# cure-lab/MagicDrive

Hardware: NVIDIA H100
Metric: 6-view 224x400 denoising-steps/sec (higher is better)
Workload: dtype bf16

## Files before the change

### magicdrive_b200/csrc/attention_wgmma.cuh

```cuda
#pragma once
#include "ptx.cuh"
#include "wgmma.cuh"

namespace mdb {

constexpr int ATT_BM = 128;

constexpr int ATT_MAX_SRC = 3;
struct AttnKvMaps {
  CUtensorMap k[ATT_MAX_SRC], v[ATT_MAX_SRC];
};

struct AttnParams {
  void* out;
  int ldo;
  int lq, lk;
  const int* kv_index;
  int n_sets;
  const int* kv_len;
  int n_src;
  float scale_log2;
  int q_step;
};

template <int D, int BN_ = 0>
struct AttnCfg {
  static constexpr int KD = (D + 63) / 64;
  static constexpr int D16 = (D + 15) / 16 * 16;
  static constexpr int BN = BN_ ? BN_ : ((D16 <= 64) ? 128 : 64);
  static constexpr int TILE_Q = ATT_BM * 128;
  static constexpr int TILE_KV = BN * 128;
  static constexpr int SMEM_Q = KD * TILE_Q;
  static constexpr int STAGES_FIT = (232448 - 1024 - 256 - SMEM_Q) / (2 * KD * TILE_KV);
  static constexpr int STAGES = STAGES_FIT > 4 ? 4 : STAGES_FIT;
  static constexpr int SMEM_KV = STAGES * 2 * KD * TILE_KV;
  static constexpr int kSmemBytes = SMEM_Q + SMEM_KV + 1024 + 256;
  static constexpr int kConsumerWarps = 8;
  static constexpr int kThreads = 32 * kConsumerWarps + 32;
  static constexpr int SACC = BN / 2;
  static constexpr int OACC = D16 / 2;
  static_assert(STAGES >= 1 && kSmemBytes <= 232448, "shared memory");
};

template <int D, int BN_, bool CAUSAL = false, bool KVRES = false, bool F16 = false>
__global__ void __launch_bounds__(AttnCfg<D, BN_>::kThreads, 1)
attention_wgmma_kernel(const __grid_constant__ CUtensorMap tmQ, const __grid_constant__ AttnKvMaps kvm, const AttnParams p) {
  using Cfg = AttnCfg<D, BN_>;
  using A = Act<F16>;
  using Elt = typename A::T;
  constexpr int KD = Cfg::KD, D16 = Cfg::D16, BN = Cfg::BN, STAGES = Cfg::STAGES;
  constexpr int TILE_Q = Cfg::TILE_Q, TILE_KV = Cfg::TILE_KV;
  extern __shared__ uint8_t smem_raw[];
  uint8_t* smem = reinterpret_cast<uint8_t*>((reinterpret_cast<uintptr_t>(smem_raw) + 1023) & ~uintptr_t(1023));
  uint8_t* smQ = smem;
  uint8_t* smK = smQ + Cfg::SMEM_Q;
  uint8_t* smV = smK + STAGES * KD * TILE_KV;
  uint64_t* bars = reinterpret_cast<uint64_t*>(smV + STAGES * KD * TILE_KV);
  uint64_t* q_full = bars;
  uint64_t* q_empty = bars + 1;
  uint64_t* kv_full = bars + 2;
  uint64_t* kv_empty = bars + 2 + STAGES;

  const int warp = threadIdx.x >> 5, lane = threadIdx.x & 31;
  const int b = blockIdx.z, head = blockIdx.y;
  const int nq = (p.lq + ATT_BM - 1) / ATT_BM;
  const int q_step = p.q_step > 0 ? p.q_step : nq;
  const int n_own = (nq - static_cast<int>(blockIdx.x) + q_step - 1) / q_step;
  auto q0_of = [&](int o) { return (static_cast<int>(blockIdx.x) + o * q_step) * ATT_BM; };

  if (warp == Cfg::kConsumerWarps && lane == 0) {
    prefetch_tmap(&tmQ);
    for (int i = 0; i < p.n_src; ++i) {
      prefetch_tmap(&kvm.k[i]);
      prefetch_tmap(&kvm.v[i]);
    }
    mbar_init(q_full, 1);
    mbar_init(q_empty, Cfg::kConsumerWarps);
    for (int i = 0; i < STAGES; ++i) {
      mbar_init(&kv_full[i], 1);
      mbar_init(&kv_empty[i], Cfg::kConsumerWarps);
    }
    fence_barrier_init();
  }
  __syncthreads();
  asm volatile("griddepcontrol.wait;" ::: "memory");
  asm volatile("griddepcontrol.launch_dependents;" ::: "memory");
  const int lkb = p.kv_len ? min(max(p.kv_len[b], 0), p.lk) : p.lk;
  const int ntiles = (lkb + BN - 1) / BN;
  static_assert(!(CAUSAL && KVRES), "resident key tiles: every query tile walks all of them");
  const bool kv_resident = (KVRES ? ntiles <= STAGES : ntiles == 1) && p.n_sets == 1 && n_own > 1;
  auto kv_entry = [&](int set) { return p.kv_index ? p.kv_index[b * p.n_sets + set] : b; };
  auto tiles_of = [&](int kve, int q0) {
    return kve < 0 ? 0 : CAUSAL ? min(ntiles, (min(q0 + ATT_BM, p.lq) - 1) / BN + 1) : ntiles;
  };

  if (warp == Cfg::kConsumerWarps) {
    if (lane == 0) {
      int stage = 0;
      uint32_t phase = 0;
      for (int o = 0; o < n_own; ++o) {
        if (o > 0) mbar_wait(q_empty, static_cast<uint32_t>(o - 1) & 1u);
        mbar_arrive_expect_tx(q_full, KD * TILE_Q);
#pragma unroll
        for (int c = 0; c < KD; ++c) tma_load_4d(&tmQ, q_full, smQ + c * TILE_Q, c * 64, head, q0_of(o), b);
        if (kv_resident && o > 0) continue;
        for (int set = 0; set < p.n_sets; ++set) {
          const int kve = kv_entry(set);
          const int nt = tiles_of(kve, q0_of(o));
          if (nt == 0) continue;
          const int kvb = kve & 0xffffff;
          const CUtensorMap* km = &kvm.k[kve >> 24];
          const CUtensorMap* vm = &kvm.v[kve >> 24];
          for (int j = 0; j < nt; ++j) {
            mbar_wait(&kv_empty[stage], phase ^ 1);
            mbar_arrive_expect_tx(&kv_full[stage], 2 * KD * TILE_KV);
#pragma unroll
            for (int c = 0; c < KD; ++c) {
              tma_load_4d(km, &kv_full[stage], smK + (stage * KD + c) * TILE_KV, c * 64, head, j * BN, kvb);
              tma_load_4d(vm, &kv_full[stage], smV + (stage * KD + c) * TILE_KV, c * 64, head, j * BN, kvb);
            }
            if (++stage == STAGES) {
              stage = 0;
              phase ^= 1;
            }
          }
        }
      }
    }
    return;
  }

  const int wg = warp >> 2;
  const int q = lane & 3;
  const int rloc = 64 * wg + 16 * (warp & 3) + (lane >> 2);
  const float sc = p.scale_log2;
  int stage = 0;
  uint32_t phase = 0;
  for (int o = 0; o < n_own; ++o) {
    const int q0 = q0_of(o);
    mbar_wait(q_full, static_cast<uint32_t>(o) & 1u);
    bool wrote = false;
    for (int set = 0; set < p.n_sets; ++set) {
      const int nt = tiles_of(kv_entry(set), q0);
      if (nt == 0) continue;
      float oacc[Cfg::OACC];
#pragma unroll
      for (int i = 0; i < Cfg::OACC; ++i) oacc[i] = 0.f;
      float m[2] = {-INFINITY, -INFINITY}, l[2] = {0.f, 0.f};
      for (int j = 0; j < nt; ++j) {
        const int st = kv_resident ? (KVRES ? j : 0) : stage;
        mbar_wait(&kv_full[st], kv_resident ? 0u : phase);
        float s[Cfg::SACC];
        wgmma_fence();
#pragma unroll
        for (int k = 0; k < D16 / 16; ++k) {
          const int c = k / 4, kk = k % 4;
          const uint64_t adesc = make_sw128_kmajor_desc(smem_u32(smQ + c * TILE_Q + wg * (64 * 128))) + 2 * kk;
          const uint64_t bdesc = make_sw128_kmajor_desc(smem_u32(smK + (st * KD + c) * TILE_KV)) + 2 * kk;
          WgmmaSS<BN, F16>::run(s, adesc, bdesc, k > 0 ? 1u : 0u);
        }
        wgmma_commit();
        wgmma_wait<0>();
        const int kbase = j * BN;
        if (kbase + BN > lkb) {
#pragma unroll
          for (int g = 0; g < BN / 8; ++g)
#pragma unroll
            for (int e = 0; e < 2; ++e)
              if (kbase + 8 * g + 2 * q + e >= lkb) s[4 * g + e] = s[4 * g + 2 + e] = -INFINITY;
        }
        if constexpr (CAUSAL) {
          if (kbase + BN - 1 > q0 + rloc) {
#pragma unroll
            for (int g = 0; g < BN / 8; ++g)
#pragma unroll
              for (int h = 0; h < 2; ++h)
#pragma unroll
                for (int e = 0; e < 2; ++e)
                  if (kbase + 8 * g + 2 * q + e > q0 + rloc + 8 * h) s[4 * g + 2 * h + e] = -INFINITY;
          }
        }
        float corr[2];
#pragma unroll
        for (int h = 0; h < 2; ++h) {
          float mx = -INFINITY;
#pragma unroll
          for (int g = 0; g < BN / 8; ++g) mx = fmaxf(mx, fmaxf(s[4 * g + 2 * h], s[4 * g + 2 * h + 1]));
          mx = fmaxf(mx, __shfl_xor_sync(0xffffffffu, mx, 1));
          mx = fmaxf(mx, __shfl_xor_sync(0xffffffffu, mx, 2));
          const float m_new = fmaxf(m[h], mx * sc);
          corr[h] = exp2f(m[h] - m_new);
          m[h] = m_new;
        }
        uint32_t pa[BN / 16][4];
        float rs[2] = {0.f, 0.f};
#pragma unroll
        for (int kk = 0; kk < BN / 16; ++kk) {
#pragma unroll
          for (int r = 0; r < 4; ++r) {
            const int h = r & 1;
            const int i0 = 8 * kk + 4 * (r >> 1) + 2 * h;
            const float p0 = exp2f(fmaf(s[i0], sc, -m[h]));
            const float p1 = exp2f(fmaf(s[i0 + 1], sc, -m[h]));
            rs[h] += p0 + p1;
            pa[kk][r] = A::pack(p0, p1);
          }
        }
#pragma unroll
        for (int h = 0; h < 2; ++h) l[h] = l[h] * corr[h] + rs[h];
#pragma unroll
        for (int g = 0; g < D16 / 8; ++g) {
          oacc[4 * g] *= corr[0], oacc[4 * g + 1] *= corr[0];
          oacc[4 * g + 2] *= corr[1], oacc[4 * g + 3] *= corr[1];
        }
        wgmma_fence();
#pragma unroll
        for (int kk = 0; kk < BN / 16; ++kk) {
          const uint64_t bdesc = make_sw128_mnmajor_desc(smem_u32(smV + st * KD * TILE_KV), TILE_KV) + (2048u >> 4) * kk;
          WgmmaRSBmn<D16, F16>::run(oacc, pa[kk], bdesc, 1u);
        }
        wgmma_commit();
        wgmma_wait<0>();
        if (!kv_resident) {
          if (lane == 0) mbar_arrive(&kv_empty[stage]);
          if (++stage == STAGES) {
            stage = 0;
            phase ^= 1;
          }
        }
      }
#pragma unroll
      for (int h = 0; h < 2; ++h) {
        l[h] += __shfl_xor_sync(0xffffffffu, l[h], 1);
        l[h] += __shfl_xor_sync(0xffffffffu, l[h], 2);
      }
      const float inv[2] = {1.0f / l[0], 1.0f / l[1]};
#pragma unroll
      for (int h = 0; h < 2; ++h) {
        const int qrow = q0 + rloc + 8 * h;
        if (qrow >= p.lq) continue;
        Elt* orow = static_cast<Elt*>(p.out) + (static_cast<long long>(b) * p.lq + qrow) * p.ldo + head * D;
#pragma unroll
        for (int g = 0; g < D16 / 8; ++g) {
          const int col = 8 * g + 2 * q;
          if (col >= D) continue;
          float f0 = oacc[4 * g + 2 * h] * inv[h], f1 = oacc[4 * g + 2 * h + 1] * inv[h];
          if (wrote) {
            const float2 pf = A::to_float2(*reinterpret_cast<const typename A::T2*>(orow + col));
            f0 = A::to_float(A::from_float(f0)) + pf.x;
            f1 = A::to_float(A::from_float(f1)) + pf.y;
          }
          *reinterpret_cast<uint32_t*>(orow + col) = A::pack(f0, f1);
        }
      }
      wrote = true;
    }
    if (!wrote) {
#pragma unroll
      for (int h = 0; h < 2; ++h) {
        const int qrow = q0 + rloc + 8 * h;
        if (qrow >= p.lq) continue;
        Elt* orow = static_cast<Elt*>(p.out) + (static_cast<long long>(b) * p.lq + qrow) * p.ldo + head * D;
#pragma unroll
        for (int g = 0; g < D16 / 8; ++g)
          if (8 * g + 2 * q < D) *reinterpret_cast<uint32_t*>(orow + 8 * g + 2 * q) = 0u;
      }
    }
    __syncwarp();
    if (lane == 0) mbar_arrive(q_empty);
  }
}

}
```

### magicdrive_b200/csrc/capi_attention.cu

```cuda
#include <cuda_bf16.h>
#include <cuda_runtime.h>

#include <stdlib.h>
#include <string.h>

#include "../../include/magicdrive_b200.h"
#define MDB_NEED_TENSORMAP
#include "common_host.h"
#include "attention_wgmma.cuh"

namespace {

bool make_qkv_map(CUtensorMap* m, const void* ptr, int d, int heads, int l, int b, int ld, int rows, bool f16) {
  mdb::EncodeTiledFn enc = mdb::get_encode();
  if (!enc) return false;
  cuuint64_t dims[4] = {(cuuint64_t)d, (cuuint64_t)heads, (cuuint64_t)l, (cuuint64_t)b};
  cuuint64_t strides[3] = {(cuuint64_t)d * 2, (cuuint64_t)ld * 2, (cuuint64_t)l * ld * 2};
  cuuint32_t box[4] = {64u, 1u, (cuuint32_t)rows, 1u};
  cuuint32_t estr[4] = {1u, 1u, 1u, 1u};
  return enc(m, f16 ? CU_TENSOR_MAP_DATA_TYPE_FLOAT16 : CU_TENSOR_MAP_DATA_TYPE_BFLOAT16, 4, const_cast<void*>(ptr), dims, strides, box, estr,
             CU_TENSOR_MAP_INTERLEAVE_NONE, CU_TENSOR_MAP_SWIZZLE_128B, CU_TENSOR_MAP_L2_PROMOTION_L2_256B,
             CU_TENSOR_MAP_FLOAT_OOB_FILL_NONE) == CUDA_SUCCESS;
}

struct KvSources {
  const void* k[mdb::ATT_MAX_SRC];
  const void* v[mdb::ATT_MAX_SRC];
  int ldk[mdb::ATT_MAX_SRC], ldv[mdb::ATT_MAX_SRC], b_kv[mdb::ATT_MAX_SRC];
  int n;
};

bool make_kv_maps(mdb::AttnKvMaps* m, const KvSources& s, int d, int heads, int lk, int rows, bool f16) {
  for (int i = 0; i < mdb::ATT_MAX_SRC; ++i) {
    const int j = i < s.n ? i : 0;
    if (!make_qkv_map(&m->k[i], s.k[j], d, heads, lk, s.b_kv[j], s.ldk[j], rows, f16) ||
        !make_qkv_map(&m->v[i], s.v[j], d, heads, lk, s.b_kv[j], s.ldv[j], rows, f16))
      return false;
  }
  return true;
}

int attn_num_sms() {
  static int sms = 0;
  if (!sms) {
    int dev = 0;
    cudaGetDevice(&dev);
    if (cudaDeviceGetAttribute(&sms, cudaDevAttrMultiProcessorCount, dev) != cudaSuccess || sms <= 0) sms = 132;
  }
  return sms;
}

int multi_q_step(int b, int heads, int lq, int lk, int n_sets, int bn, bool resident) {
  if ((lk > bn && !resident) || n_sets != 1) return 0;
  const char* e = getenv("MDB_ATTN_MULTIQ");
  if (e && e[0] == '0') return 0;
  const int nq = (lq + mdb::ATT_BM - 1) / mdb::ATT_BM;
  const long long per_tile_ctas = static_cast<long long>(b) * heads;
  const long long slots = attn_num_sms();
  if (per_tile_ctas * nq <= slots) return 0;
  long long gx = slots / per_tile_ctas;
  if (gx < 1) gx = 1;
  if (gx >= nq) return 0;
  return static_cast<int>(gx);
}

constexpr int ATT_RESIDENT_MAX_LK = 256;

template <int D, int BN_, bool CAUSAL, bool KVRES = false, bool F16 = false>
int launch_attention(const void* q, int ldq, const KvSources& src, void* out, int ldo, int b, int heads, int lq, int lk,
                     const int* kv_index, int n_sets, const int* kv_len, float scale, cudaStream_t st) {
  using Cfg = mdb::AttnCfg<D, BN_>;
  if constexpr (!CAUSAL && !KVRES) {
    if (kv_len && n_sets == 1 && lk <= ATT_RESIDENT_MAX_LK)
      return launch_attention<D, BN_, false, true, F16>(q, ldq, src, out, ldo, b, heads, lq, lk, kv_index, n_sets, kv_len, scale, st);
  }
  static bool attr = false;
  if (!attr) {
    cudaError_t e = cudaFuncSetAttribute(mdb::attention_wgmma_kernel<D, BN_, CAUSAL, KVRES, F16>, cudaFuncAttributeMaxDynamicSharedMemorySize, Cfg::kSmemBytes);
    if (e != cudaSuccess) return mdb::set_error(MDB_ERR_CUDA, "attention_wgmma_kernel smem attr: %s", cudaGetErrorString(e));
    attr = true;
  }
  CUtensorMap tq;
  mdb::AttnKvMaps kvm;
  if (!make_qkv_map(&tq, q, D, heads, lq, b, ldq, mdb::ATT_BM, F16) || !make_kv_maps(&kvm, src, D, heads, lk, Cfg::BN, F16))
    return mdb::set_error(MDB_ERR_CUDA, "mdb_attention: cuTensorMapEncodeTiled failed (d=%d heads=%d lq=%d lk=%d)", D, heads, lq, lk);
  mdb::AttnParams p;
  p.out = out;
  p.ldo = ldo, p.lq = lq, p.lk = lk, p.kv_index = kv_index, p.n_sets = n_sets, p.kv_len = kv_len, p.n_src = src.n;
  p.scale_log2 = scale * 1.4426950408889634f;
  p.q_step = multi_q_step(b, heads, lq, lk, n_sets, Cfg::BN, KVRES);
  dim3 grid(p.q_step > 0 ? p.q_step : (lq + mdb::ATT_BM - 1) / mdb::ATT_BM, heads, b);
  cudaError_t le = mdb::launch_pdl(mdb::attention_wgmma_kernel<D, BN_, CAUSAL, KVRES, F16>, grid, dim3(Cfg::kThreads), Cfg::kSmemBytes, st, tq, kvm, p);
  if (le != cudaSuccess) return mdb::set_error(MDB_ERR_CUDA, "attention_wgmma_kernel launch: %s", cudaGetErrorString(le));
  cudaError_t e2 = cudaGetLastError();
  if (e2 != cudaSuccess) return mdb::set_error(MDB_ERR_CUDA, "attention_wgmma_kernel: %s", cudaGetErrorString(e2));
  return MDB_OK;
}

template <int BN_, bool CAUSAL, bool F16 = false>
int attention_dispatch_bn(const void* q, int ldq, const KvSources& src, void* out, int ldo, int b, int heads, int lq, int lk, int d,
                          const int* kv_index, int n_sets, const int* kv_len, float scale, cudaStream_t st) {
  switch (d) {
    case 32: return launch_attention<32, BN_, CAUSAL, false, F16>(q, ldq, src, out, ldo, b, heads, lq, lk, kv_index, n_sets, kv_len, scale, st);
    case 40: return launch_attention<40, BN_, CAUSAL, false, F16>(q, ldq, src, out, ldo, b, heads, lq, lk, kv_index, n_sets, kv_len, scale, st);
    case 64: return launch_attention<64, BN_, CAUSAL, false, F16>(q, ldq, src, out, ldo, b, heads, lq, lk, kv_index, n_sets, kv_len, scale, st);
    case 80: return launch_attention<80, BN_, CAUSAL, false, F16>(q, ldq, src, out, ldo, b, heads, lq, lk, kv_index, n_sets, kv_len, scale, st);
    case 160: return launch_attention<160, BN_, CAUSAL, false, F16>(q, ldq, src, out, ldo, b, heads, lq, lk, kv_index, n_sets, kv_len, scale, st);
    default: return mdb::set_error(MDB_ERR_UNSUPPORTED, "mdb_attention: head dim %d not instantiated (32, 40, 64, 80, 160)", d);
  }
}

template <bool CAUSAL = false>
int attention_dispatch(const void* q, int ldq, const KvSources& src, void* out, int ldo, int b, int heads, int lq, int lk, int d,
                       const int* kv_index, int n_sets, const int* kv_len, float scale, cudaStream_t st) {
  const char* e = getenv("MDB_ATTN_KERNEL");
  if (e && !strcmp(e, "tc2d")) return attention_dispatch_bn<64, CAUSAL>(q, ldq, src, out, ldo, b, heads, lq, lk, d, kv_index, n_sets, kv_len, scale, st);
  if (e && !strcmp(e, "tc")) return attention_dispatch_bn<128, CAUSAL>(q, ldq, src, out, ldo, b, heads, lq, lk, d, kv_index, n_sets, kv_len, scale, st);
  if (e && *e && strcmp(e, "tc2"))
    return mdb::set_error(MDB_ERR_INVALID, "mdb_attention: MDB_ATTN_KERNEL must be tc2, tc2d or tc (got %s)", e);
  return attention_dispatch_bn<0, CAUSAL>(q, ldq, src, out, ldo, b, heads, lq, lk, d, kv_index, n_sets, kv_len, scale, st);
}

template <bool F16>
int attention_varlen(const void* q, int ldq, int n_src, const void* const* k, const int* ldk, const void* const* v,
                     const int* ldv, const int* b_kv, void* out, int ldo, int b, int heads, int lq, int lk, int d,
                     const int* kv_index, int n_sets, const int* kv_len, float scale, void* stream) {
  using namespace mdb;
  if (!q || !k || !v || !ldk || !ldv || !b_kv || !out) return set_error(MDB_ERR_INVALID, "mdb_attention: null pointer");
  if (n_src < 1 || n_src > ATT_MAX_SRC) return set_error(MDB_ERR_INVALID, "mdb_attention: 1..%d K/V sources", ATT_MAX_SRC);
  if (n_sets < 1 || n_sets > MDB_ATT_MAX_SETS || (n_sets > 1 && !kv_index))
    return set_error(MDB_ERR_INVALID, "mdb_attention: n_sets must be 1..%d (more than 1 needs kv_index)", MDB_ATT_MAX_SETS);
  if (scale <= 0.f) return set_error(MDB_ERR_INVALID, "mdb_attention: scale must be positive");
  if (lq <= 0 || lk <= 0 || b <= 0 || heads <= 0) return set_error(MDB_ERR_INVALID, "mdb_attention: bad shape");
  if (ldq % 8 || ldo % 8) return set_error(MDB_ERR_UNSUPPORTED, "mdb_attention: strides must be multiples of 8");
  KvSources src;
  src.n = n_src;
  for (int i = 0; i < n_src; ++i) {
    if (!k[i] || !v[i] || b_kv[i] <= 0) return set_error(MDB_ERR_INVALID, "mdb_attention: bad K/V source %d", i);
    if (ldk[i] % 8 || ldv[i] % 8) return set_error(MDB_ERR_UNSUPPORTED, "mdb_attention: strides must be multiples of 8");
    src.k[i] = k[i], src.v[i] = v[i], src.ldk[i] = ldk[i], src.ldv[i] = ldv[i], src.b_kv[i] = b_kv[i];
  }
  if (!kv_index && (n_src != 1 || b_kv[0] != b)) return set_error(MDB_ERR_INVALID, "mdb_attention: b_kv != b or several sources need kv_index");
  if constexpr (F16) {
    return attention_dispatch_bn<0, false, true>(q, ldq, src, out, ldo, b, heads, lq, lk, d, kv_index, n_sets, kv_len, scale,
                                                 static_cast<cudaStream_t>(stream));
  } else {
    return attention_dispatch(q, ldq, src, out, ldo, b, heads, lq, lk, d, kv_index, n_sets, kv_len, scale,
                              static_cast<cudaStream_t>(stream));
  }
}

}

extern "C" int mdb_attention_varlen(const void* q, int ldq, int n_src, const void* const* k, const int* ldk, const void* const* v,
                                    const int* ldv, const int* b_kv, void* out, int ldo, int b, int heads, int lq, int lk, int d,
                                    const int* kv_index, int n_sets, const int* kv_len, float scale, void* stream) {
  return attention_varlen<false>(q, ldq, n_src, k, ldk, v, ldv, b_kv, out, ldo, b, heads, lq, lk, d, kv_index, n_sets, kv_len,
                                 scale, stream);
}

extern "C" int mdb_attention_varlen_f16(const void* q, int ldq, int n_src, const void* const* k, const int* ldk,
                                        const void* const* v, const int* ldv, const int* b_kv, void* out, int ldo, int b, int heads,
                                        int lq, int lk, int d, const int* kv_index, int n_sets, const int* kv_len, float scale,
                                        void* stream) {
  return attention_varlen<true>(q, ldq, n_src, k, ldk, v, ldv, b_kv, out, ldo, b, heads, lq, lk, d, kv_index, n_sets, kv_len,
                                scale, stream);
}

extern "C" int mdb_attention_multi(const void* q, int ldq, int n_src, const void* const* k, const int* ldk, const void* const* v,
                                   const int* ldv, const int* b_kv, void* out, int ldo, int b, int heads, int lq, int lk, int d,
                                   const int* kv_index, int n_sets, float scale, void* stream) {
  return mdb_attention_varlen(q, ldq, n_src, k, ldk, v, ldv, b_kv, out, ldo, b, heads, lq, lk, d, kv_index, n_sets, nullptr, scale,
                              stream);
}

extern "C" int mdb_attention(const void* q, int ldq, const void* k, int ldk, const void* v, int ldv, void* out, int ldo, int b,
                             int b_kv, int heads, int lq, int lk, int d, const int* kv_index, int n_sets, float scale,
                             void* stream) {
  return mdb_attention_multi(q, ldq, 1, &k, &ldk, &v, &ldv, &b_kv, out, ldo, b, heads, lq, lk, d, kv_index, n_sets, scale, stream);
}

extern "C" int mdb_attention_causal(const void* q, int ldq, const void* k, int ldk, const void* v, int ldv, void* out, int ldo,
                                    int b, int heads, int lq, int lk, int d, float scale, void* stream) {
  using namespace mdb;
  if (!q || !k || !v || !out) return set_error(MDB_ERR_INVALID, "mdb_attention_causal: null pointer");
  if (lq != lk) return set_error(MDB_ERR_INVALID, "mdb_attention_causal: lq (%d) must equal lk (%d)", lq, lk);
  if (scale <= 0.f) return set_error(MDB_ERR_INVALID, "mdb_attention_causal: scale must be positive");
  if (lq <= 0 || b <= 0 || heads <= 0) return set_error(MDB_ERR_INVALID, "mdb_attention_causal: bad shape");
  if (ldq % 8 || ldk % 8 || ldv % 8 || ldo % 8) return set_error(MDB_ERR_UNSUPPORTED, "mdb_attention_causal: strides must be multiples of 8");
  KvSources src;
  src.n = 1;
  src.k[0] = k, src.v[0] = v, src.ldk[0] = ldk, src.ldv[0] = ldv, src.b_kv[0] = b;
  return attention_dispatch<true>(q, ldq, src, out, ldo, b, heads, lq, lk, d, nullptr, 1, nullptr, scale,
                                  static_cast<cudaStream_t>(stream));
}
```

Measured before the change: 59.06.

## Add persistent attention kernel with double-buffered Q tiles

Adds a persistent variant of the WGMMA attention kernel that launches at most one CTA per SM and walks a flattened list of (batch, head, query-tile) work items in strides. Q is double-buffered in shared memory so the producer warp can load the next tile's Q and K/V while consumers finish the current one. The goal is to cut per-CTA launch and prologue cost and hide tile-boundary latency. In exchange it drops the resident-KV reuse path for these launches, needs extra shared memory, and may balance load worse when item counts do not divide evenly across SMs.

```diff
diff --git a/magicdrive_b200/csrc/attention_wgmma.cuh b/magicdrive_b200/csrc/attention_wgmma.cuh
--- a/magicdrive_b200/csrc/attention_wgmma.cuh
+++ b/magicdrive_b200/csrc/attention_wgmma.cuh
@@ -1,6 +1,8 @@
 #pragma once
 #include "ptx.cuh"
 #include "wgmma.cuh"
+
+#include <type_traits>
 
 namespace mdb {
 
@@ -21,6 +23,9 @@
   int n_src;
   float scale_log2;
   int q_step;
+};
+struct AttnParamsPersist : AttnParams {
+  int heads, b;
 };
 
 template <int D, int BN_ = 0>
@@ -35,6 +40,7 @@
   static constexpr int STAGES = STAGES_FIT > 4 ? 4 : STAGES_FIT;
   static constexpr int SMEM_KV = STAGES * 2 * KD * TILE_KV;
   static constexpr int kSmemBytes = SMEM_Q + SMEM_KV + 1024 + 256;
+  static constexpr int kSmemBytesPersist = kSmemBytes + SMEM_Q;
   static constexpr int kConsumerWarps = 8;
   static constexpr int kThreads = 32 * kConsumerWarps + 32;
   static constexpr int SACC = BN / 2;
@@ -42,30 +48,38 @@
   static_assert(STAGES >= 1 && kSmemBytes <= 232448, "shared memory");
 };
 
-template <int D, int BN_, bool CAUSAL = false, bool KVRES = false, bool F16 = false>
+template <int D, int BN_, bool CAUSAL = false, bool KVRES = false, bool F16 = false, bool PERSIST = false>
 __global__ void __launch_bounds__(AttnCfg<D, BN_>::kThreads, 1)
-attention_wgmma_kernel(const __grid_constant__ CUtensorMap tmQ, const __grid_constant__ AttnKvMaps kvm, const AttnParams p) {
+attention_wgmma_kernel(const __grid_constant__ CUtensorMap tmQ, const __grid_constant__ AttnKvMaps kvm,
+                       const std::conditional_t<PERSIST, AttnParamsPersist, AttnParams> p) {
   using Cfg = AttnCfg<D, BN_>;
   using A = Act<F16>;
   using Elt = typename A::T;
   constexpr int KD = Cfg::KD, D16 = Cfg::D16, BN = Cfg::BN, STAGES = Cfg::STAGES;
   constexpr int TILE_Q = Cfg::TILE_Q, TILE_KV = Cfg::TILE_KV;
+  constexpr int QS = PERSIST ? 2 : 1;
+  static_assert(!PERSIST || (!CAUSAL && !KVRES && Cfg::kSmemBytesPersist <= 232448), "persistent: plain launches only");
   extern __shared__ uint8_t smem_raw[];
   uint8_t* smem = reinterpret_cast<uint8_t*>((reinterpret_cast<uintptr_t>(smem_raw) + 1023) & ~uintptr_t(1023));
   uint8_t* smQ = smem;
-  uint8_t* smK = smQ + Cfg::SMEM_Q;
+  uint8_t* smK = smQ + QS * Cfg::SMEM_Q;
   uint8_t* smV = smK + STAGES * KD * TILE_KV;
   uint64_t* bars = reinterpret_cast<uint64_t*>(smV + STAGES * KD * TILE_KV);
   uint64_t* q_full = bars;
-  uint64_t* q_empty = bars + 1;
-  uint64_t* kv_full = bars + 2;
-  uint64_t* kv_empty = bars + 2 + STAGES;
+  uint64_t* q_empty = bars + QS;
+  uint64_t* kv_full = bars + 2 * QS;
+  uint64_t* kv_empty = bars + 2 * QS + STAGES;
 
   const int warp = threadIdx.x >> 5, lane = threadIdx.x & 31;
-  const int b = blockIdx.z, head = blockIdx.y;
+  int b = blockIdx.z, head = blockIdx.y;
   const int nq = (p.lq + ATT_BM - 1) / ATT_BM;
   const int q_step = p.q_step > 0 ? p.q_step : nq;
-  const int n_own = (nq - static_cast<int>(blockIdx.x) + q_step - 1) / q_step;
+  const int n_own = [&] {
+    if constexpr (PERSIST)
+      return (nq * p.heads * p.b - static_cast<int>(blockIdx.x) + static_cast<int>(gridDim.x) - 1) / static_cast<int>(gridDim.x);
+    else
+      return (nq - static_cast<int>(blockIdx.x) + q_step - 1) / q_step;
+  }();
   auto q0_of = [&](int o) { return (static_cast<int>(blockIdx.x) + o * q_step) * ATT_BM; };
 
   if (warp == Cfg::kConsumerWarps && lane == 0) {
@@ -74,8 +88,10 @@
       prefetch_tmap(&kvm.k[i]);
       prefetch_tmap(&kvm.v[i]);
     }
-    mbar_init(q_full, 1);
-    mbar_init(q_empty, Cfg::kConsumerWarps);
+    for (int i = 0; i < QS; ++i) {
+      mbar_init(&q_full[i], 1);
+      mbar_init(&q_empty[i], Cfg::kConsumerWarps);
+    }
     for (int i = 0; i < STAGES; ++i) {
       mbar_init(&kv_full[i], 1);
       mbar_init(&kv_empty[i], Cfg::kConsumerWarps);
@@ -85,10 +101,23 @@
   __syncthreads();
   asm volatile("griddepcontrol.wait;" ::: "memory");
   asm volatile("griddepcontrol.launch_dependents;" ::: "memory");
-  const int lkb = p.kv_len ? min(max(p.kv_len[b], 0), p.lk) : p.lk;
-  const int ntiles = (lkb + BN - 1) / BN;
+  int lkb = p.kv_len ? min(max(p.kv_len[b], 0), p.lk) : p.lk;
+  int ntiles = (lkb + BN - 1) / BN;
+  auto begin_item = [&](int o) {
+    if constexpr (PERSIST) {
+      const int t = static_cast<int>(blockIdx.x) + o * static_cast<int>(gridDim.x);
+      const int bh = t / nq;
+      head = bh % p.heads;
+      b = bh / p.heads;
+      lkb = p.kv_len ? min(max(p.kv_len[b], 0), p.lk) : p.lk;
+      ntiles = (lkb + BN - 1) / BN;
+      return (t - bh * nq) * ATT_BM;
+    } else {
+      return q0_of(o);
+    }
+  };
   static_assert(!(CAUSAL && KVRES), "resident key tiles: every query tile walks all of them");
-  const bool kv_resident = (KVRES ? ntiles <= STAGES : ntiles == 1) && p.n_sets == 1 && n_own > 1;
+  const bool kv_resident = !PERSIST && (KVRES ? ntiles <= STAGES : ntiles == 1) && p.n_sets == 1 && n_own > 1;
   auto kv_entry = [&](int set) { return p.kv_index ? p.kv_index[b * p.n_sets + set] : b; };
   auto tiles_of = [&](int kve, int q0) {
     return kve < 0 ? 0 : CAUSAL ? min(ntiles, (min(q0 + ATT_BM, p.lq) - 1) / BN + 1) : ntiles;
@@ -99,14 +128,16 @@
       int stage = 0;
       uint32_t phase = 0;
       for (int o = 0; o < n_own; ++o) {
-        if (o > 0) mbar_wait(q_empty, static_cast<uint32_t>(o - 1) & 1u);
-        mbar_arrive_expect_tx(q_full, KD * TILE_Q);
-#pragma unroll
-        for (int c = 0; c < KD; ++c) tma_load_4d(&tmQ, q_full, smQ + c * TILE_Q, c * 64, head, q0_of(o), b);
+        const int qs = PERSIST ? o & 1 : 0;
+        if (o >= QS) mbar_wait(&q_empty[qs], static_cast<uint32_t>((o - QS) / QS) & 1u);
+        mbar_arrive_expect_tx(&q_full[qs], KD * TILE_Q);
+        const int q0 = begin_item(o);
+#pragma unroll
+        for (int c = 0; c < KD; ++c) tma_load_4d(&tmQ, &q_full[qs], smQ + (qs * KD + c) * TILE_Q, c * 64, head, q0, b);
         if (kv_resident && o > 0) continue;
         for (int set = 0; set < p.n_sets; ++set) {
           const int kve = kv_entry(set);
-          const int nt = tiles_of(kve, q0_of(o));
+          const int nt = tiles_of(kve, q0);
           if (nt == 0) continue;
           const int kvb = kve & 0xffffff;
           const CUtensorMap* km = &kvm.k[kve >> 24];
@@ -137,8 +168,10 @@
   int stage = 0;
   uint32_t phase = 0;
   for (int o = 0; o < n_own; ++o) {
-    const int q0 = q0_of(o);
-    mbar_wait(q_full, static_cast<uint32_t>(o) & 1u);
+    const int q0 = begin_item(o);
+    const int qs = PERSIST ? o & 1 : 0;
+    const uint8_t* smQs = smQ + qs * Cfg::SMEM_Q;
+    mbar_wait(&q_full[qs], static_cast<uint32_t>(o / QS) & 1u);
     bool wrote = false;
     for (int set = 0; set < p.n_sets; ++set) {
       const int nt = tiles_of(kv_entry(set), q0);
@@ -155,7 +188,7 @@
 #pragma unroll
         for (int k = 0; k < D16 / 16; ++k) {
           const int c = k / 4, kk = k % 4;
-          const uint64_t adesc = make_sw128_kmajor_desc(smem_u32(smQ + c * TILE_Q + wg * (64 * 128))) + 2 * kk;
+          const uint64_t adesc = make_sw128_kmajor_desc(smem_u32(smQs + c * TILE_Q + wg * (64 * 128))) + 2 * kk;
           const uint64_t bdesc = make_sw128_kmajor_desc(smem_u32(smK + (st * KD + c) * TILE_KV)) + 2 * kk;
           WgmmaSS<BN, F16>::run(s, adesc, bdesc, k > 0 ? 1u : 0u);
         }
@@ -267,7 +300,7 @@
       }
     }
     __syncwarp();
-    if (lane == 0) mbar_arrive(q_empty);
+    if (lane == 0) mbar_arrive(&q_empty[qs]);
   }
 }
 
diff --git a/magicdrive_b200/csrc/capi_attention.cu b/magicdrive_b200/csrc/capi_attention.cu
--- a/magicdrive_b200/csrc/capi_attention.cu
+++ b/magicdrive_b200/csrc/capi_attention.cu
@@ -1,6 +1,7 @@
 #include <cuda_bf16.h>
 #include <cuda_runtime.h>
 
+#include <limits.h>
 #include <stdlib.h>
 #include <string.h>
 
@@ -66,6 +67,31 @@
 
 constexpr int ATT_RESIDENT_MAX_LK = 256;
 
+template <int D, int BN_, bool CAUSAL, bool KVRES>
+constexpr bool kHasPersistent = !CAUSAL && !KVRES && BN_ == 0 && D <= 80;
+
+template <int D, int BN_, bool CAUSAL, bool KVRES, bool F16>
+cudaError_t launch_persistent(int items, int heads, int b, const CUtensorMap& tq, const mdb::AttnKvMaps& kvm,
+                              const mdb::AttnParams& p, cudaStream_t st) {
+  if constexpr (!kHasPersistent<D, BN_, CAUSAL, KVRES>) {
+    return cudaErrorNotSupported;
+  } else {
+    using Cfg = mdb::AttnCfg<D, BN_>;
+    constexpr auto kernel = mdb::attention_wgmma_kernel<D, BN_, false, false, F16, true>;
+    static bool attr = false;
+    if (!attr) {
+      cudaError_t e = cudaFuncSetAttribute(kernel, cudaFuncAttributeMaxDynamicSharedMemorySize, Cfg::kSmemBytesPersist);
+      if (e != cudaSuccess) return e;
+      attr = true;
+    }
+    mdb::AttnParamsPersist pp;
+    static_cast<mdb::AttnParams&>(pp) = p;
+    pp.heads = heads, pp.b = b;
+    const int grid = items < attn_num_sms() ? items : attn_num_sms();
+    return mdb::launch_pdl(kernel, dim3(grid), dim3(Cfg::kThreads), Cfg::kSmemBytesPersist, st, tq, kvm, pp);
+  }
+}
+
 template <int D, int BN_, bool CAUSAL, bool KVRES = false, bool F16 = false>
 int launch_attention(const void* q, int ldq, const KvSources& src, void* out, int ldo, int b, int heads, int lq, int lk,
                      const int* kv_index, int n_sets, const int* kv_len, float scale, cudaStream_t st) {
@@ -89,8 +115,16 @@
   p.ldo = ldo, p.lq = lq, p.lk = lk, p.kv_index = kv_index, p.n_sets = n_sets, p.kv_len = kv_len, p.n_src = src.n;
   p.scale_log2 = scale * 1.4426950408889634f;
   p.q_step = multi_q_step(b, heads, lq, lk, n_sets, Cfg::BN, KVRES);
-  dim3 grid(p.q_step > 0 ? p.q_step : (lq + mdb::ATT_BM - 1) / mdb::ATT_BM, heads, b);
-  cudaError_t le = mdb::launch_pdl(mdb::attention_wgmma_kernel<D, BN_, CAUSAL, KVRES, F16>, grid, dim3(Cfg::kThreads), Cfg::kSmemBytes, st, tq, kvm, p);
+  const int nq = (lq + mdb::ATT_BM - 1) / mdb::ATT_BM;
+  cudaError_t le;
+  if (kHasPersistent<D, BN_, CAUSAL, KVRES> && p.q_step == 0) {
+    const long long items = static_cast<long long>(nq) * heads * b;
+    if (items > INT_MAX) return mdb::set_error(MDB_ERR_UNSUPPORTED, "mdb_attention: %lld work items", items);
+    le = launch_persistent<D, BN_, CAUSAL, KVRES, F16>(static_cast<int>(items), heads, b, tq, kvm, p, st);
+  } else {
+    dim3 grid(p.q_step > 0 ? p.q_step : nq, heads, b);
+    le = mdb::launch_pdl(mdb::attention_wgmma_kernel<D, BN_, CAUSAL, KVRES, F16>, grid, dim3(Cfg::kThreads), Cfg::kSmemBytes, st, tq, kvm, p);
+  }
   if (le != cudaSuccess) return mdb::set_error(MDB_ERR_CUDA, "attention_wgmma_kernel launch: %s", cudaGetErrorString(le));
   cudaError_t e2 = cudaGetLastError();
   if (e2 != cudaSuccess) return mdb::set_error(MDB_ERR_CUDA, "attention_wgmma_kernel: %s", cudaGetErrorString(e2));
```

Measured after the change: 59.85 (median of 6 runs). +1.3%, better.
